# THU-luvision/TextureFusion

Measured on AMD Instinct MI355X. Metric: RGB-D frames/s (TSDF integrate + atlas update: prepare->integrate->finalize, UpdateMeshes, GeneratePatches + UpdateAtlas over the frame's dirty chunks), higher is better.
Workload: dtype f32

## Files before the change

### texturefusion_amd/csrc/tf_kernels.hip

```cpp
#include <stdlib.h>

#include <atomic>
#include "tf_device.h"
#include "tf_devfn.h"
#include "tf_host_math.h"
#include "tf_patch_body.h"
#include "tf_voxel_math.h"

#pragma clang fp contract(off)
#ifndef TF_KA_GP
#define TF_KA_GP 2
#endif


namespace tf {

__global__ void k_reset_ctl(FrameCtl* ctl, VolCtl* vctl) {
  if (blockIdx.x == 0 && threadIdx.x == 0) {
    for (int a = 0; a < 3; ++a) {
      ctl->bbox_key[a] = f2key(1e8f);
      ctl->bbox_key[3 + a] = f2key(-1e8f);
      ctl->min_id[a] = ctl->max_id[a] = ctl->dims[a] = 0;
    }
    ctl->n_coarse = 0;
// ... 497 lines not shown
  auto item_pos = [&](const uint32_t e) -> uint32_t { return FUSED ? list_phys(v, e, nf) : e; };
  const int vy = lane >> 3;
  const int W = cam.W, H = cam.H;
  if (FUSED && bid == 0 && threadIdx.x == 0) {
    for (int a = 0; a < 3; ++a) {
      L.ctl->bbox_key[a] = f2key(1e8f);
      L.ctl->bbox_key[3 + a] = f2key(-1e8f);
    }
  }

  const uint32_t e_first = wave, e_step = nwaves;
  u32x8 rec_next;
  {
    const uint32_t e0 = e_first < n_items ? e_first : 0u;
    const uint32_t p0 = n_items ? item_pos(e0) : 0u;
    rec_next = *(const_u32x8_ptr)(unsigned long long)(&L.list_pre[4 * (p0 < v.max_list ? p0 : 0u)]);
  }

  __shared__ float cenT[3][kChunkVoxels];
  {
    const float4* src = reinterpret_cast<const float4*>(L.cen);
    float4* dst = reinterpret_cast<float4*>(&cenT[0][0]);
    for (int i = threadIdx.x; i < 3 * kChunkVoxels / 4; i += 256) dst[i] = src[i];
  }
  __syncthreads();

  const __amdgpu_buffer_rsrc_t rs_depth =
      __builtin_amdgcn_make_buffer_rsrc((void*)img.depth, 0, W * H * 4, 0x00020000);
  const __amdgpu_buffer_rsrc_t rs_rgba =
      __builtin_amdgcn_make_buffer_rsrc((void*)img.rgba, 0, COLOR ? W * H * 4 : 0, 0x00020000);
  const __amdgpu_buffer_rsrc_t rs_qual =
      __builtin_amdgcn_make_buffer_rsrc((void*)img.quality, 0, QUALITY ? W * H * 4 : 0, 0x00020000);

  const uint32_t row_lo = lane < 32 ? (0xFFu << (lane & 24)) : 0u;
  const uint32_t row_hi = lane < 32 ? 0u : (0xFFu << (lane & 24));
  auto row_any = [&](const unsigned long long m) -> bool {
    return ((((uint32_t)m) & row_lo) | (((uint32_t)(m >> 32)) & row_hi)) != 0u;
  };
  auto ballot = [](const bool b) -> unsigned long long { return __builtin_amdgcn_ballot_w64(b); };

  float c_near = cam.nearP, c_far = cam.farP, c_thr = kc.thrCol, c_lower = kc.lower, c_sigma = kc.sigma;
  asm volatile("" : "+v"(c_near), "+v"(c_far), "+v"(c_thr), "+v"(c_lower), "+v"(c_sigma));

  if (TL && (kc.dbg & 8192u) && lane == 0 && wave < (uint32_t)kPhaseWaves)
  {
    v.phase_buf[wave * 16 + 14] = __builtin_amdgcn_s_memrealtime();
    v.phase_buf[wave * 16 + 8] = 0;
    v.phase_buf[wave * 16 + 9] = 0;
  }

  for (uint32_t e = e_first, e_next = e_first + e_step; e < n_items; e = e_next) {
    const uint32_t pe = item_pos(e);
    const u32x8 prw = rec_next;
    {
      e_next = e + e_step;
      const uint32_t en = e_next < n_items ? e_next : e;
      rec_next = *(const_u32x8_ptr)(unsigned long long)(&L.list_pre[4 * item_pos(en)]);
    }
    const int4 id = make_int4((int)prw[5], (int)prw[6], (int)prw[7], 0);
    const bool owned = part_owned(v, id.x, id.y, id.z);
    if (!owned) {
      if (FUSED && lane == 0) {
        L.list_slot[pe] = kInvalidSlot; L.list_ent[pe] = 0; L.list_new[pe] = 0; L.list_needs[pe] = 0;
        L.list_quality[pe] = 0.0f; L.list_rows[pe] = 0;
      }
      continue;
    }
    const unsigned long long key = pack_id(id.x, id.y, id.z);
    const uint32_t i0 = hash_key(key) & v.hmask;
    u32x4 h0 = {0u, 0u, 0u, 0u};
    uint32_t slot = kInvalidSlot;
    if (FUSED) h0 = *(const_u32x4_ptr)(unsigned long long)(&v.hent[i0]);
    else slot = L.list_slot[pe];
    bool is_new = false;
    uint32_t ent = i0;

    const float o0 = __uint_as_float(prw[0]), o1 = __uint_as_float(prw[1]), o2 = __uint_as_float(prw[2]);
    const float pbx = __uint_as_float(prw[3]), pby = __uint_as_float(prw[4]);
    const f32x2 o01 = {o0, o1};
    const f32x2 fxy = {cam.fxi, cam.fyi}, cxy = {kc.cxs, kc.cys};
    const float wD = FLAG ? pbx : -pbx;
    const float upper = pby;
    const float band = 32.0f * kc.res;
    const bool div_safe = (fabsf(o2) > band) && (fabsf(o2) < 1048576.0f) && (fabsf(o0) < 1048576.0f) &&
                          (fabsf(o1) < 1048576.0f) && (kc.res > 1e-6f) && (kc.res < 16.0f);
    if (TL && (kc.dbg & 8192u) && e == e_first && lane == 0 && wave < (uint32_t)kPhaseWaves) {
      asm volatile("" :: "s"(o0), "s"(o1), "s"(o2), "s"(id.x));
      v.phase_buf[wave * 16 + 15] = __builtin_amdgcn_s_memrealtime();
    }

    int off_d[8];
    int oobl[QUALITY ? 8 : 1];
    int oob_any = 0;
    uint32_t R = 64;
    unsigned long long all_valid = ~0ull;
    uint32_t oob_bits = 0;
    auto geometry = [&](auto safe_tag) {
      constexpr bool SAFE = decltype(safe_tag)::value;
#pragma unroll
      for (int j = 0; j < 8; ++j) {
        const int k = j * 64 + lane;
        const f32x2 pxy = o01 + (f32x2){cenT[0][k], cenT[1][k]};
        const float pzv = o2 + cenT[2][k];
        f32x2 q;
        if (SAFE) {
          q = div2_by(pxy, recip_refined(pzv));
        } else {
          q.x = pxy.x / pzv;
          q.y = pxy.y / pzv;
        }
        const f32x2 uw = q * fxy + cxy;
        const int X = SAFE ? cvt_rne_hw(uw.x) : cvt_sat_rne(uw.x);
        const int Y = SAFE ? cvt_rne_hw(uw.y) : cvt_sat_rne(uw.y);
        const bool valid = ((unsigned)(X - 1) < (unsigned)(W - 2)) && ((unsigned)(Y - 1) < (unsigned)(H - 2));
        all_valid &= ballot(valid);
        int od = (__mul24(Y, W) + X) * 4;
        asm volatile("" : "+v"(od));
        off_d[j] = valid ? od : kOOB;
        if (COLOR) oob_bits |= (((unsigned)X > (unsigned)(W - 1)) || ((unsigned)Y > (unsigned)(H - 1))) ? (1u << j) : 0u;
      }
    };
    if (div_safe) geometry(std::true_type{});
    else geometry(std::false_type{});
    if (QUALITY) {
#pragma unroll
      for (int j = 0; j < 8; ++j) oobl[j] = 0;
    }
    if (all_valid != ~0ull) {
#pragma unroll
      for (int j = 0; j < 8; ++j) {
        if (R == 64u) {
          const unsigned long long vmj = ballot(off_d[j] != kOOB);
          const unsigned long long dead = nonzero_bytes(vmj) ^ 0x0101010101010101ull;
          if (dead) R = (uint32_t)(j * 8) + ((uint32_t)__builtin_ctzll(dead) >> 3);
        }
        const bool live_lane = (uint32_t)(j * 8 + vy) < R;
        if (COLOR) {
          const bool oob = live_lane && ((oob_bits >> j) & 1u);
          oob_any |= oob ? 1 : 0;
          if (QUALITY) oobl[j] = oob ? 1 : 0;
        }
        off_d[j] = live_lane ? off_d[j] : kOOB;
      }
    }

    float dep[8];
#pragma unroll
    for (int j = 0; j < 8; ++j)
      dep[j] = __uint_as_float(__builtin_amdgcn_raw_buffer_load_b32(rs_depth, off_d[j], 0, 0));

    bool lazy_revive = false;
    if (FUSED) {
      if ((((unsigned long long)h0.y << 32) | h0.x) == key && h0.z != kInvalidSlot) {
        slot = h0.z;
        is_new = lazy_revive = (h0.w == 0u);
      } else {
        uint32_t s0 = kInvalidSlot, nw = 1, en = 0;
        if (lane == 0) {
          bool bnew = true;
          s0 = chunk_acquire(v, id, &bnew, &en);
          nw = bnew ? 1u : 0u;
        }
        slot = (uint32_t)__builtin_amdgcn_readfirstlane((int)s0);
        is_new = __builtin_amdgcn_readfirstlane((int)nw) != 0;
        ent = (uint32_t)__builtin_amdgcn_readfirstlane((int)en);
      }
    }
    if (slot == kInvalidSlot) {
      if (FUSED && lane == 0) {
        L.list_slot[pe] = kInvalidSlot; L.list_ent[pe] = 0; L.list_new[pe] = 0; L.list_needs[pe] = 0;
        L.list_quality[pe] = 0.0f; L.list_rows[pe] = 0;
      }
      continue;
    }
    const __amdgpu_buffer_rsrc_t rs_T =
        __builtin_amdgcn_make_buffer_rsrc((void*)(v.tsdf + (size_t)slot * kChunkVoxels), 0, 4096, 0x00020000);
    const __amdgpu_buffer_rsrc_t rs_C =
        __builtin_amdgcn_make_buffer_rsrc((void*)(v.color + (size_t)slot * kChunkVoxels), 0, 4096, 0x00020000);

    float qsum = 0.0f;
    uint32_t lanes_t = 0, lanes_c = 0;
    uint32_t sword = 0;
    unsigned long long m_ok = 0, m_pos = 0, m_neg = 0, m_hvy = 0;

#pragma unroll
    for (int p = 0; p < 8 / GP; ++p) {
      const int g0 = p * GP;
      if ((uint32_t)(g0 * 8) >= R) break;
      float nwv[GP], sd[GP];
      int off_t[GP], off_c[GP], off_i[GP];
      unsigned long long any = 0ull;
#pragma unroll
      for (int j = 0; j < GP; ++j) {
        const int gj = g0 + j;
        const int kb = (gj * 64 + lane) * 8;
        const float d = dep[gj];
        const float s = d - (o2 + cenT[2][gj * 64 + lane]);
        sd[j] = s;
        if (COLOR) {
          const bool upd = (off_d[gj] != kOOB) && (fabsf(s) < c_thr);
          off_i[j] = upd ? off_d[gj] : kOOB;
          const bool ru_l = row_any(ballot(upd));
          const unsigned long long ru = ballot(ru_l);
          off_c[j] = ru_l ? kb : kOOB;
          lanes_c += (uint32_t)__popcll(ru);
          any |= ru;
        }
        const bool act = (uint32_t)(gj * 8 + vy) < R;
        const bool dv = (d > c_near) && (c_far > d);
        const bool inside = (s > c_lower) && (upper > s);
        const bool F = act && dv && inside;
        nwv[j] = F ? wD : 0.0f;
        const bool rf_l = row_any(ballot(F));
        const unsigned long long rf = ballot(rf_l);
        off_t[j] = rf_l ? kb : kOOB;
        lanes_t += (uint32_t)__popcll(rf);
        any |= rf;
      }
      const bool rmw = (any != 0ull) || (COLOR && QUALITY);
      u32x2 t[GP], c[GP];
      uint32_t in[GP];
      float qv[GP];
      if (rmw) {
#pragma unroll
        for (int j = 0; j < GP; ++j) t[j] = __builtin_amdgcn_raw_buffer_load_b64(rs_T, off_t[j], 0, 0);
        if (COLOR) {
#pragma unroll
          for (int j = 0; j < GP; ++j) {
            c[j] = __builtin_amdgcn_raw_buffer_load_b64(rs_C, off_c[j], 0, 0);
            in[j] = __builtin_amdgcn_raw_buffer_load_b32(rs_rgba, off_i[j], 0, 0);
            if (QUALITY) qv[j] = __uint_as_float(__builtin_amdgcn_raw_buffer_load_b32(rs_qual, off_i[j], 0, 0));
          }
        }
      }
      if (rmw) {
#pragma unroll
        for (int j = 0; j < GP; ++j) {
          if (COLOR) {
            const uint32_t p_rg = __builtin_amdgcn_perm(0u, in[j], 0x0c010c00u);
            const uint32_t p_ba = __builtin_amdgcn_perm(0u, in[j], 0x0c030c02u);
            const uint32_t w_rg = c[j].x, w_ba = c[j].y;
            const u16x2 in_rg = __builtin_bit_cast(u16x2, p_rg), in_ba = __builtin_bit_cast(u16x2, p_ba);
            u16x2 c_rg = __builtin_bit_cast(u16x2, w_rg), c_ba = __builtin_bit_cast(u16x2, w_ba);
            if (FLAG) {
              c_rg += in_rg;
              c_ba += in_ba;
              const bool halve = (int)__builtin_bit_cast(uint32_t, c_ba) >= (121 << 16);
              const u16x2 h_rg = c_rg >> (unsigned short)2, h_ba = c_ba >> (unsigned short)2;
              c_rg = halve ? h_rg : c_rg;
              c_ba = halve ? h_ba : c_ba;
            } else {
              c_rg -= in_rg;
              c_ba -= in_ba;
            }
            c[j].x = __builtin_bit_cast(uint32_t, c_rg);
            c[j].y = __builtin_bit_cast(uint32_t, c_ba);
          }
          const float ts = __uint_as_float(t[j].x), tw = __uint_as_float(t[j].y);
          const float nw = nwv[j];
          const float num = ts * tw + sd[j] * nw;
          const float den = (tw + nw) + c_sigma;
          const float ns = num / den;
          const float nwt = tw + nw;
          const bool keep = nwt > 0.5f;
          t[j].x = __float_as_uint(keep ? ns : 999.0f);
          t[j].y = __float_as_uint(keep ? nwt : 0.0f);
        }
      }
      if (rmw) {
#pragma unroll
        for (int j = 0; j < GP; ++j) {
          if (COLOR) __builtin_amdgcn_raw_buffer_store_b64(c[j], rs_C, off_c[j], 0, 0);
          __builtin_amdgcn_raw_buffer_store_b64(t[j], rs_T, off_t[j], 0, 0);
          if (!(kc.dbg & kKaCoarseSumm)) {
            const float fs = __uint_as_float(t[j].x), fw = __uint_as_float(t[j].y);
            const unsigned long long b_ok = ballot(!(fs > 1.0f)), b_pos = ballot(fs > 0.0f) & b_ok;
            const unsigned long long b_neg = ballot(fs < 0.0f), b_hvy = ballot(fw > 50.0f);
            m_ok |= b_ok; m_pos |= b_pos; m_neg |= b_neg; m_hvy |= b_hvy;
            if (g0 + j == 0)
              sword = (b_ok ? 0x1000u : 0u) | (b_pos ? 0x2000u : 0u) | (b_neg ? 0x4000u : 0u) | (b_hvy ? 0x8000u : 0u);
          }
        }
      }
      if (COLOR && QUALITY) {
        const int rowshift = lane & 56;
#pragma unroll
        for (int j = 0; j < GP; ++j) {
          const int gj = g0 + j;
          const unsigned long long mu = ballot(off_i[j] != kOOB);
          const unsigned long long mo = ballot(oobl[gj] != 0);
          if ((mu | mo) == 0ull) continue;
          float rowsum = 0.0f;
          if (mu) {
#pragma unroll
            for (int l = 0; l < 8; ++l) rowsum += __shfl(qv[j], rowshift + l);
          }
          const int left = (int)R - gj * 8;
          const int rmax = left < 8 ? left : 8;
          for (int r = 0; r < rmax; ++r) {
            if ((mo >> (8 * r)) & 0xFFull) qsum = kc.qoob;
            if ((mu >> (8 * r)) & 0xFFull)
              qsum += __int_as_float(__builtin_amdgcn_readlane(__float_as_int(rowsum), 8 * r));
          }
        }
      }
    }
    const uint32_t rows_t = lanes_t >> 3, rows_c = COLOR ? (lanes_c >> 3) : 0u;
    const bool updated = rows_t != 0;
    if (updated) {
      if (kc.dbg & kKaCoarseSumm) {
        if (lane == 0) v.summ[slot] = kSummAny;
      } else {
        const unsigned long long mm[4] = {m_ok, m_pos, m_neg, m_hvy};
#pragma unroll
        for (int b = 0; b < 4; ++b)
          sword |= (mm[b] ? (1u << b) : 0u) | ((mm[b] & 0x0101010101010101ull) ? (0x10u << b) : 0u) | ((mm[b] & 0xFFull) ? (0x100u << b) : 0u);
        if (lane == 0 && sword) atomicOr(&v.summ[slot], sword);
      }
    }
    if (TL && (kc.dbg & 8192u) && lane == 0 && wave < (uint32_t)kPhaseWaves) {
      v.phase_buf[wave * 16 + 8] += 1;
      v.phase_buf[wave * 16 + 9] += rows_t + rows_c;
    }
    if (COLOR && !QUALITY) {
      if (ballot(oob_any != 0) != 0ull) qsum = kc.qoob;
    }

    const bool face = part_band(v, id.x, id.y, id.z);
    if (updated && lane == 0 && (face || lazy_revive)) {
      const uint32_t en = FUSED ? ent : L.list_ent[pe];
      if (face) mark_touched(v, en);
      else v.hent[en].alive = 1u;
    }
    if (FUSED) {
      if (updated) {
        if (lane == 0) v.mark_epoch[slot] = epoch + 1u;
        if (claim_par >= 0) {
          claim_dirty7(v, id, slot, ent, lane, epoch + 1u, claim_par);
        }
      } else if (is_new) {
        if (lane == 0) {
          if (!lazy_revive) v.hent[ent].alive = 0;
          v.mark_epoch[(size_t)v.max_chunks + slot] = epoch + 1u;
        }
        if (rows_c) {
          uint4* c4 = reinterpret_cast<uint4*>(v.color + (size_t)slot * kChunkVoxels);
#pragma unroll
          for (int k = 0; k < 4; ++k) c4[k * 64 + lane] = make_uint4(0, 0, 0, 0);
        }
      }
      if (lane == 0) {
        L.list_slot[pe] = slot;
        L.list_needs[pe] = updated ? 1 : 0;
        L.list_rows[pe] = (uint16_t)(rows_t | (rows_c << 8));
      }
    } else if (lane == 0) {
      if (updated) L.list_needs[pe] = 1;
      L.list_quality[pe] = qsum;
      L.list_rows[pe] = (uint16_t)(rows_t | (rows_c << 8));
    }
  }
}

template <bool COLOR, bool QUALITY, bool FLAG>
__global__ __launch_bounds__(256) void k_integrate(VolumeDev v, FrameImages img, Cam cam, IntegrateConsts kc,
                                                   uint32_t epoch) {
  integrate_body<COLOR, QUALITY, false, FLAG, TF_KA_GP>(v, img, cam, kc, epoch, blockIdx.x, gridDim.x);
}

struct FrameLaunch {
  VolumeDev v;
  FrameImages img;
  Pose P;
  IntegrateConsts kc;
  Cam cam;
  Integ ig;
  uint32_t epoch;
  uint32_t n_ka, n_sel, n_bbox;
  uint32_t rot;
  SelBuf sel1;
  const float* depth1;
  SelectConsts sc1;
  FrameCtl* ctl2;
  const float* depth2;
  Pose P2;
  int claim_par;
  uint32_t n_patch;
  int patch_par;
  KfDev kf_patch;
  uint32_t* progress;
  uint32_t progress_val;
};

template <bool COLOR, bool PATCH, bool TL = false>
__global__ __launch_bounds__(256) __attribute__((amdgpu_waves_per_eu(PATCH ? TF_KFP_WAVES : TF_KF_WAVES, PATCH ? TF_KFP_WAVES : TF_KF_WAVES))) void k_frame(FrameLaunch a) {
  const uint32_t total = a.n_ka + a.n_patch + a.n_sel + a.n_bbox;
  const uint32_t b = blockIdx.x + a.rot < total ? blockIdx.x + a.rot : blockIdx.x + a.rot - total;
  const bool timeline = TL && (a.kc.dbg & 4096u) != 0 && a.n_sel > 0 && a.n_bbox > 0;
  const unsigned long long t0 = timeline ? __builtin_amdgcn_s_memrealtime() : 0ull;
  uint32_t role;
  if (b < a.n_ka) {
    role = 0;
    integrate_body<COLOR, false, true, true, TF_KA_GP, TL>(a.v, a.img, a.cam, a.kc, a.epoch, b, a.n_ka, a.claim_par);
  } else if (PATCH && b < a.n_ka + a.n_patch) {
    role = 3;
    patch_body<true, true, true, TL>(a.v, a.cam, a.patch_par, a.kf_patch, b - a.n_ka, a.n_patch);
  } else if (b < a.n_ka + a.n_patch + a.n_sel) {
    role = 1;
    if (!(TL && (a.kc.dbg & 512u))) {
      VolumeDev v1 = a.v;
      v1.sel = a.sel1;
      select_body<true>(a.depth1, a.cam, a.ig, a.sc1, v1, b - a.n_ka - a.n_patch, a.n_sel);
    }
  } else {
    role = 2;
    if (a.progress && b + 1 == total && threadIdx.x == 0)
      __hip_atomic_store(a.progress, a.progress_val, __ATOMIC_RELAXED, __HIP_MEMORY_SCOPE_SYSTEM);
    if (!(TL && (a.kc.dbg & 1024u))) bbox_body(a.depth2, a.cam, a.P2, a.ctl2, b - a.n_ka - a.n_patch - a.n_sel, a.n_bbox);
  }
// ... 486 lines not shown
```

### texturefusion_amd/csrc/tf_mesh.hip

```cpp
#include <stdlib.h>
#include <string.h>

#include <algorithm>
#include <vector>

#include "tf_devfn.h"
#include "tf_kf_store.h"
#include "tf_mc_table.h"
#include "tf_patch_body.h"
#include "tf_volume.h"

#pragma clang fp contract(off)

namespace tf {

__device__ const unsigned long long d_mc_tri[256] = TF_MC_TRI_TABLE_INIT;

constexpr int kR = 11;
constexpr int kRS = 11;
constexpr int kPS = kRS * kR;
constexpr int kRV = kPS * kR;
constexpr int kEdgeSlots = 3 * 729;
__device__ __forceinline__ uint32_t mesh_shard_rows_d(uint32_t max_chunks) { return max_chunks / kMeshShards + 258u; }

__device__ __forceinline__ int ridx(int x, int y, int z) { return (x + 1) + (y + 1) * kRS + (z + 1) * kPS; }

constexpr bool halo_needed(int rx, int ry, int rz) {
  if (rx < -1 || rx > 9 || ry < -1 || ry > 9 || rz < -1 || rz > 9) return false;
  if (rx >= 0 && rx < 8 && ry >= 0 && ry < 8 && rz >= 0 && rz < 8) return false;
  const int out = ((rx < 0 || rx > 8) ? 1 : 0) + ((ry < 0 || ry > 8) ? 1 : 0) + ((rz < 0 || rz > 8) ? 1 : 0);
  return out <= 1;
}
constexpr int count_halo_pairs() {
  int n = 0;
  for (int rz = -1; rz <= 9; ++rz)
    for (int ry = -1; ry <= 9; ++ry)
      for (int rx = -1; rx <= 9; ++rx) {
        if (!halo_needed(rx, ry, rz)) continue;
        const int vx = (rx + 8) & 7;
        if ((vx & 1) && halo_needed(rx - 1, ry, rz) && (((rx - 1 + 8) >> 3) == ((rx + 8) >> 3))) continue;
        ++n;
      }
  return n;
}
constexpr int kHalo = count_halo_pairs();
struct MeshTabs {
  unsigned long long halo[kHalo];
  uint16_t corner[729];
};
constexpr unsigned long long corner_of(int rx, int ry, int rz) {
  return (rx >= 0 && ry >= 0 && rz >= 0 && rx <= 8 && ry <= 8 && rz <= 8) ? (unsigned long long)(rx + ry * 9 + rz * 81 + 1) : 0ull;
}
constexpr MeshTabs make_mesh_tabs() {
  MeshTabs t{};
  int n = 0;
  for (int rz = -1; rz <= 9; ++rz)
    for (int ry = -1; ry <= 9; ++ry)
      for (int rx = -1; rx <= 9; ++rx) {
        if (!halo_needed(rx, ry, rz)) continue;
        const int vx = (rx + 8) & 7;
        const bool same_chunk_left = ((rx - 1 + 8) >> 3) == ((rx + 8) >> 3);
        if ((vx & 1) && halo_needed(rx - 1, ry, rz) && same_chunk_left) continue;
        const int rx0 = (vx & 1) ? rx - 1 : rx;
        const bool use0 = !(vx & 1);
        const bool use1 = (vx & 1) ? true : (halo_needed(rx + 1, ry, rz) && (((rx + 1 + 8) >> 3) == ((rx + 8) >> 3)));
        const int cx = (rx + 8) >> 3, cy = (ry + 8) >> 3, cz = (rz + 8) >> 3;
        const unsigned long long nb = (unsigned long long)(cx + cy * 3 + cz * 9);
        const unsigned long long pair = (unsigned long long)((((rx0 + 8) & 7) + ((ry + 8) & 7) * 8 + ((rz + 8) & 7) * 64) >> 1);
        const unsigned long long r0 = (unsigned long long)((rx0 + 1) + (ry + 1) * kRS + (rz + 1) * kPS);
        t.halo[n++] = (r0 & 2047ull) | (nb << 11) | (pair << 16) | ((use0 ? 1ull : 0ull) << 24) | ((use1 ? 1ull : 0ull) << 25) |
                      ((use0 ? corner_of(rx0, ry, rz) : 0ull) << 26) | ((use1 ? corner_of(rx0 + 1, ry, rz) : 0ull) << 36);
      }
  for (int c = 0; c < 729; ++c) {
    const int px = c % 9, py = (c / 9) % 9, pz = c / 81;
    t.corner[c] = (uint16_t)((px + 1) + (py + 1) * kRS + (pz + 1) * kPS);
  }
  return t;
}
__device__ const MeshTabs d_mesh_tabs = make_mesh_tabs();

__device__ __forceinline__ int cox(int k) { return (0x66 >> k) & 1; }
__device__ __forceinline__ int coy(int k) { return (0xCC >> k) & 1; }
__device__ __forceinline__ int coz(int k) { return (0xF0 >> k) & 1; }
__device__ __forceinline__ int edge_c0(int e) { return (int)((0x321076543210ull >> (4 * e)) & 0xF); }
__device__ __forceinline__ int edge_c1(int e) { return (int)((0x765447650321ull >> (4 * e)) & 0xF); }

__device__ __forceinline__ int edge_slot(int x, int y, int z, int e) {
  const int bx = x + ((0x622 >> e) & 1);
  const int by = y + ((0xC44 >> e) & 1);
  const int bz = z + ((0x0F0 >> e) & 1);
  const int ax = e >= 8 ? 2 : (e & 1);
  return ax + (bx + by * 9 + bz * 81) * 3;
}
__device__ __forceinline__ int edge_of_slot(int ax, int dx, int dy, int dz) {
  if (ax == 0) return dz ? (dy ? 6 : 4) : (dy ? 2 : 0);
  if (ax == 1) return dz ? (dx ? 5 : 7) : (dx ? 1 : 3);
  return dy ? (dx ? 10 : 11) : (dx ? 9 : 8);
}

__device__ __forceinline__ bool gradient_at(const float* __restrict__ S, int px, int py, int pz, int ox, int oy,
                                            int oz, float res, float g[3]) {
  const int c = ridx(px, py, pz);
  const float xm = S[c - 1], xp = S[c + 1];
  const float ym = S[c - kRS], yp = S[c + kRS];
  const float zm = S[c - kPS], zp = S[c + kPS];
  const bool ok = ((ox ? xp : xm) < 1.0f) && ((oy ? yp : ym) < 1.0f) && ((oz ? zp : zm) < 1.0f);
  const float gx = xp - xm, gy = yp - ym, gz = zp - zm;
  const float yz = gy * gy + gz * gz;
  const float sq = gx * gx + yz;
  const float n = sqrtf(sq);
  g[0] = gx; g[1] = gy; g[2] = gz;
  if (sq > 0.0f) { g[0] = gx / n; g[1] = gy / n; g[2] = gz / n; }
  return ok && !(n > res * 100.0f);
}

constexpr uint32_t kCfHeavy = 64u;
constexpr uint32_t kCfGradOk = 128u;

template <int NT>
struct MeshSh {
  float S[kRV];
  uint8_t cflag[732];
  uint32_t nslot[27];
  unsigned long long rmask[NT];
  uint16_t rbase[NT];
  uint32_t ownq[(kEdgeSlots + 7) / 8];
  uint16_t cinfo[512];
  uint8_t cidx[512];
  uint16_t toff[512];
  uint32_t wsum[8];
  uint32_t nv, nt, adj, any;
  uint32_t ncell;
  uint16_t clist[512];
  uint32_t ovf;
  uint32_t rblock;
  uint32_t rpress;
  uint32_t rstate;
  unsigned long long rtexloc;
};

__device__ __forceinline__ int edge_q(int e) {
  return (int)((0x231023320110ull >> (4 * e)) & 0x3);
}
__device__ __forceinline__ int owner_cell(int m, int q) {
  const int ax = m % 3, b = m / 3;
  const int bx = b % 9, by = (b / 9) % 9, bz = b / 81;
  const int d0 = q & 1, d1 = q >> 1;
  int x, y, z;
  if (ax == 0) { x = bx; y = by - d0; z = bz - d1; }
  else if (ax == 1) { x = bx - d0; y = by; z = bz - d1; }
  else { x = bx - d0; y = by - d1; z = bz; }
  return x + 8 * y + 64 * z;
}

__device__ __forceinline__ void patch_list_append(const VolumeDev& v, int ppar, uint32_t shard, const int4 id,
                                                  uint32_t slot, unsigned long long texloc, uint32_t blk) {
  const uint32_t rows = mesh_shard_rows_d(v.max_chunks);
  const uint32_t p = atomicAdd(&v.patch_cnt[((ppar & 1) * kMeshShards + shard) * 16], 1u);
  const unsigned long long key = pack_id(id.x, id.y, id.z);
  if (p < rows) v.patch_list[((size_t)(ppar & 1) * kMeshShards + shard) * rows + p] = make_int4((int)(uint32_t)key, (int)(uint32_t)(key >> 32), (int)slot, (int)blk);
  else atomicOr(&v.vctl->status, kStMeshFull);
  if (texloc == kNoTexloc) {
    const uint32_t c = atomicAdd(&v.actl->set[ppar & 1].n_cand, 1u);
    if (c < v.max_chunks) v.cand[c] = pack_id(id.x, id.y, id.z);
  }
// ... 320 lines not shown
template <int NT, bool DBG = false>
__global__ __launch_bounds__(NT, TF_MESH_WAVES) void k_mesh(VolumeDev v, const uint32_t* __restrict__ surv, uint32_t* __restrict__ cnt,
                                                 uint32_t* __restrict__ cnt_next, uint32_t cap_sh,
                                                 uint32_t epoch, float res, uint32_t simplified, uint32_t dbg,
                                                 int rearm) {
  __shared__ MeshSh<NT> sh;
  extern __shared__ uint16_t vlist[];
  const int t = threadIdx.x, lane = t & 63;
  uint32_t n_rows = 0, excl_l = 0, incl_l = 0;
  {
    uint32_t my_n = cnt[(lane & 31) * 16 + (lane >> 5)];
    if (my_n > cap_sh) my_n = cap_sh;
    uint32_t incl = my_n;
#pragma unroll
    for (int o = 1; o < 64; o <<= 1) {
      const uint32_t u = (uint32_t)__shfl_up((int)incl, o);
      if (lane >= o) incl += u;
    }
    n_rows = (uint32_t)__builtin_amdgcn_readfirstlane(__shfl((int)incl, 63));
    const uint32_t r0 = blockIdx.x;
    const uint32_t sh0 = (uint32_t)__popcll(__ballot(incl <= r0));
    incl_l = (uint32_t)__builtin_amdgcn_readfirstlane(__shfl((int)incl, (int)(sh0 & 63u)));
    excl_l = incl_l - (uint32_t)__builtin_amdgcn_readfirstlane(__shfl((int)my_n, (int)(sh0 & 63u)));
    incl_l = (uint32_t)__builtin_amdgcn_readfirstlane((int)sh0);
  }
  if (blockIdx.x == 0 && t < (int)kMeshShards) { cnt_next[t * 16] = 0u; cnt_next[t * 16 + 1] = 0u; cnt_next[(kMeshShards + t) * 16] = 0u; cnt_next[(kMeshShards + t) * 16 + 1] = 0u; cnt_next[(2 * kMeshShards + t) * 16] = 0u; }
  if (blockIdx.x < kMeshShards) {
    uint32_t n_reset = cnt[(2u * kMeshShards + blockIdx.x) * 16u];
    if (n_reset > cap_sh) n_reset = cap_sh;
    for (uint32_t i = (uint32_t)t; i < n_reset; i += NT) {
      const int4 e = v.reset_list[(size_t)blockIdx.x * cap_sh + i];
      filter_reset_record(v, (uint32_t)e.w, make_int4(e.x, e.y, e.z, 0), epoch, rearm >= 0 ? (rearm ^ 1) : -1);
    }
  }
  const float half = res * 0.5f;
  if (rearm >= 0 && blockIdx.x == 0 && t == 0) {
    AtlasCtl::Set* O = &v.actl->set[rearm];
    O->n_work = 0; O->n_cand = 0; O->n_patch = 0; O->slots_base = 0ull;
    v.actl->set[rearm ^ 1].slots_base = v.actl->n_slots;
  }
  if (rearm >= 0 && blockIdx.x == 0 && t < (int)kMeshShards) {
    v.patch_cnt[((rearm & 1) * kMeshShards + t) * 16] = 0u;
    v.wl_cnt[((rearm & 1) * kMeshShards + t) * 16] = 0u;
  }
  if (DBG && dbg == 9) mesh_stamp(v, blockIdx.x, 0);
  for (uint32_t r = blockIdx.x; r < n_rows; r += gridDim.x) {
    uint32_t shard, own;
    int4 id;
    float2 a[512 / NT];
    {
      shard = incl_l;
      uint32_t idx = r - excl_l;
      if (r != blockIdx.x) {
        uint32_t my_n = cnt[(lane & 31) * 16 + (lane >> 5)];
        if (my_n > cap_sh) my_n = cap_sh;
        uint32_t incl = my_n;
#pragma unroll
        for (int o = 1; o < 64; o <<= 1) {
          const uint32_t u = (uint32_t)__shfl_up((int)incl, o);
          if (lane >= o) incl += u;
        }
        shard = (uint32_t)__builtin_amdgcn_readfirstlane((int)__popcll(__ballot(incl <= r)));
        idx = r - (uint32_t)__builtin_amdgcn_readfirstlane(__shfl((int)incl, (int)(shard & 63u)) - __shfl((int)my_n, (int)(shard & 63u)));
      }
      if (shard >= kMeshShards) { shard -= kMeshShards; idx = cap_sh - 1u - idx; }
      const size_t row = (size_t)shard * cap_sh + idx;
      own = surv[32 * row + 13];
      id = make_int4((int)surv[32 * row + 27], (int)surv[32 * row + 28], (int)surv[32 * row + 29], 0);
#pragma unroll
      for (int j = 0; j < 512 / NT; ++j) a[j] = v.tsdf[(size_t)own * kChunkVoxels + j * NT + t];
      __syncthreads();
      if (t < 27) sh.nslot[t] = surv[32 * row + t];
    }
    int t_ = threadIdx.x;
    asm volatile("" : "+v"(t_));
    const int t = t_, lane = t & 63, w = t >> 6;
    MeshRec* rec = &v.mesh_rec[own];
    unsigned long long htab[(kHalo + NT - 1) / NT];
#pragma unroll
    for (int j = 0; j < (kHalo + NT - 1) / NT; ++j) htab[j] = (j * NT + t < kHalo) ? d_mesh_tabs.halo[j * NT + t] : ~0ull;
    if (DBG && dbg == 9) mesh_stamp(v, r, 1);
    if (t == 0) { sh.nv = 0; sh.nt = 0; sh.adj = 0; sh.ncell = 0; }
    if (t == NT - 64) { sh.rstate = rec->state; sh.rblock = rec->block; sh.rtexloc = rec->texloc; sh.rpress = blk_pressure(v); }
    if (DBG && dbg == 1) continue;
#pragma unroll
    for (int j = 0; j < 512 / NT; ++j) {
      const int q = j * NT + t;
      const int x0 = q & 7, y0 = (q >> 3) & 7, z0 = q >> 6;
      sh.S[ridx(x0, y0, z0)] = a[j].x; sh.cflag[x0 + y0 * 9 + z0 * 81] = (a[j].y > 50.0f) ? kCfHeavy : 0u;
    }
    __syncthreads();
#pragma unroll
    for (int j = 0; j < (kHalo + NT - 1) / NT; ++j) {
      const unsigned long long e = htab[j];
      if (e == ~0ull) continue;
      const uint32_t s = sh.nslot[(uint32_t)(e >> 11) & 31u];
      float4 val = make_float4(999.0f, 0.0f, 999.0f, 0.0f);
      if (s != kInvalidSlot) val = reinterpret_cast<const float4*>(v.tsdf + (size_t)s * kChunkVoxels)[(uint32_t)(e >> 16) & 255u];
      const uint32_t r0 = (uint32_t)e & 2047u;
      if ((e >> 24) & 1ull) {
        sh.S[r0] = val.x;
        const uint32_t cf = (uint32_t)(e >> 26) & 1023u;
        if (cf) sh.cflag[cf - 1u] = (val.y > 50.0f) ? kCfHeavy : 0u;
      }
      if ((e >> 25) & 1ull) {
        sh.S[r0 + 1u] = val.z;
// ... 155 lines not shown
    const uint32_t nv = sh.nv, nt = sh.nt;
    const uint32_t ovf = sh.ovf;
    if (ovf == kBlkFail) {
      if (t == 0) {
        atomicOr(&v.vctl->status, kStMeshFull);
        const uint32_t was = sh.rstate & kMsInMap;
        rec->nv = 0; rec->nt = 0; rec->state = was | kMsOverflow; rec->epoch = epoch;
        if (rearm >= 0 && was) patch_list_append(v, rearm ^ 1, shard, id, own, sh.rtexloc, sh.rblock);
      }
      __syncthreads();
      continue;
    }
    const uint16_t* const gvlist = (ovf & kBlkLarge) ? v.ovf_vlist + (size_t)((ovf & ~kBlkLarge) - 1u) * kOvfCV : nullptr;

    if (DBG && dbg == 4) continue;
    if (DBG && dbg == 9) mesh_stamp(v, r, 6);
    const uint32_t inmap = (sh.rstate & kMsInMap) | (nv ? kMsInMap : 0u);
    if (t == NT - 64) {
      mesh_block_settle(v, sh.rblock, ovf);
      if (rearm >= 0 && inmap) patch_list_append(v, rearm ^ 1, shard, id, own, sh.rtexloc, ovf);
    }
    const float org[3] = {(float)(8 * id.x) * res, (float)(8 * id.y) * res, (float)(8 * id.z) * res};
    uint32_t adj = 0;
    for (uint32_t i = t; i < nv; i += NT) {
      const int m = gvlist ? gvlist[i] : vlist[i];
      const int cell = owner_cell(m, __builtin_ctz((sh.ownq[m >> 3] >> (4 * (m & 7))) & 0xFu));
      const int x = cell & 7, y = (cell >> 3) & 7, z = cell >> 6;
      const int ax = m % 3, b = m / 3;
      const int bx = b % 9, by = (b / 9) % 9, bz = b / 81;
      const int e = edge_of_slot(ax, bx - x, by - y, bz - z);
      const int e0 = edge_c0(e), e1 = edge_c1(e);
      const float s0 = sh.S[ridx(x + cox(e0), y + coy(e0), z + coz(e0))];
      const float s1 = sh.S[ridx(x + cox(e1), y + coy(e1), z + coz(e1))];
      const float tt = s0 / (s0 - s1);
      const int o0[3] = {cox(e0), coy(e0), coz(e0)}, o1[3] = {cox(e1), coy(e1), coz(e1)};
      const int cc[3] = {x, y, z};
      float pv[3];
#pragma unroll
      for (int a = 0; a < 3; ++a) {
        const float p0 = (float)o0[a] * res, p1 = (float)o1[a] * res;
        const float ev = p0 + tt * (p1 - p0);
        const float origin = org[a] + ((float)cc[a] * res + half);
        pv[a] = ev + origin;
      }
      const int k = (fabsf(s0) > fabsf(s1)) ? e1 : e0;
      const int px = x + cox(k), py = y + coy(k), pz = z + coz(k);
      float g[3];
      gradient_at(sh.S, px, py, pz, cox(k), coy(k), coz(k), res, g);
      const uint32_t cs = sh.nslot[((px + 8) >> 3) + ((py + 8) >> 3) * 3 + ((pz + 8) >> 3) * 9];
      const ushort4 c4 = v.color[(size_t)cs * kChunkVoxels + (px & 7) + (py & 7) * 8 + (pz & 7) * 64];
      float col[3] = {1.0f, 1.0f, 1.0f};
      const float cw = (float)c4.w;
      if (cw > 0.0f) {
        col[0] = ((float)c4.x / 255.0f) / cw;
        col[1] = ((float)c4.y / 255.0f) / cw;
        col[2] = ((float)c4.z / 255.0f) / cw;
      }
#pragma unroll
      for (int a = 0; a < 3; ++a) {
        mesh_plane(v, ovf, kMpPos + a)[i] = pv[a];
        mesh_plane(v, ovf, kMpNrm + a)[i] = g[a];
        mesh_plane(v, ovf, kMpCol + a)[i] = col[a];
        const int gp = (int)floorf((pv[a] - org[a]) / (res * 1.0f));
        if (gp >= 8) adj |= 1u << (2 * a + 1);
        if (gp <= 0) adj |= 1u << (2 * a);
      }
    }
    if (adj) atomicOr(&sh.adj, adj);
    if (DBG && dbg == 9) mesh_stamp(v, r, 7);
    for (uint32_t ci = (uint32_t)(NT - 1 - t); ci < sh.ncell; ci += NT) {
      const int cell = sh.clist[ci];
      const uint32_t info = sh.cinfo[cell];
      if (!(info >> 12)) continue;
      const int x = cell & 7, y = (cell >> 3) & 7, z = cell >> 6;
      const unsigned long long row = d_mc_tri[sh.cidx[cell]];
      const uint32_t valid = info & 0xFFFu;
      uint32_t o = sh.toff[cell];
      for (int col = 0; col < 15; col += 3) {
        const int s0 = (int)((row >> (4 * col)) & 0xF);
        if (s0 == 0xF) break;
        const int s1 = (int)((row >> (4 * col + 4)) & 0xF), s2 = (int)((row >> (4 * col + 8)) & 0xF);
        if (!((valid >> s0) & (valid >> s1) & (valid >> s2) & 1u)) continue;
        constexpr int kEptT = 2304 / NT;
        auto ref_of = [&](int m) {
          const int tt = m / kEptT, j = m - tt * kEptT;
          return (uint16_t)(sh.rbase[tt] + (uint32_t)__popcll(sh.rmask[tt] & ((1ull << j) - 1ull)));
        };
        tri_plane(v, ovf, 0)[o] = ref_of(edge_slot(x, y, z, s2));
        tri_plane(v, ovf, 1)[o] = ref_of(edge_slot(x, y, z, s1));
        tri_plane(v, ovf, 2)[o] = ref_of(edge_slot(x, y, z, s0));
        ++o;
      }
    }
    __syncthreads();
    if (t == 0) {
      rec->nv = (uint16_t)nv; rec->nt = (uint16_t)nt; rec->epoch = epoch; rec->block = ovf;
      rec->state = inmap | (sh.adj << kMsAdjShift) | (inmap ? simplified : 0u);
    }
    __syncthreads();
    if (DBG && dbg == 9) mesh_stamp(v, r, 8);
  }
}

__global__ __launch_bounds__(256) void k_init_mesh_rec(MeshRec* rec, uint32_t n) {
  for (uint32_t i = blockIdx.x * 256 + threadIdx.x; i < n; i += gridDim.x * 256) {
    MeshRec r;
    memset(&r, 0, sizeof(r));
    r.texloc = kNoTexloc;
    r.frameid = -1;
    r.ratio[0] = r.ratio[1] = 1.0f;
    rec[i] = r;
  }
}
void launch_init_meshes(const VolumeDev& v, hipStream_t s) {
  hipLaunchKernelGGL(k_init_mesh_rec, dim3(1024), dim3(256), 0, s, v.mesh_rec, v.max_chunks);
  (void)hipMemsetAsync(v.mesh_rec + v.max_chunks, 0, sizeof(uint32_t) * ((size_t)blk_ring_len(v.mesh_blocks) + blk_ring_len(v.ovf_blocks)), s);
// ... 539 lines not shown
```

### texturefusion_amd/csrc/tf_voxel_math.h

```cpp
#pragma once

#include "tf_devfn.h"
#include "tf_device.h"
#include "tf_host_math.h"

#pragma clang fp contract(off)

namespace tf {

__device__ __forceinline__ int cvt_rne(float x) {
  return (x >= -2147483648.0f && x < 2147483648.0f) ? (int)rintf(x) : (int)0x80000000;
}

__device__ __forceinline__ uint32_t f2key(float f) {
  uint32_t b = __float_as_uint(f);
  return (b & 0x80000000u) ? ~b : (b | 0x80000000u);
}
__device__ __forceinline__ float key2f(uint32_t k) {
  uint32_t b = (k & 0x80000000u) ? (k & 0x7FFFFFFFu) : ~k;
  return __uint_as_float(b);
}

__device__ __forceinline__ float truncation(const Integ& ig, float z) {
  double zz = (double)z * (double)z;
// ... 53 lines not shown
    for (int a = 0; a < 3; ++a) { L.ctl->bbox_key[a] = f2key(1e8f); L.ctl->bbox_key[3 + a] = f2key(-1e8f); }
  }
  for (uint32_t e = bid * 256 + threadIdx.x; e < n; e += nb * 256) {
    const int4 id = L.list_id[e];
    bool is_new = false;
    uint32_t ent = 0;
    const uint32_t slot = chunk_acquire(v, id, &is_new, &ent, lazy);
    L.list_slot[e] = slot;
    L.list_ent[e] = ent;
    L.list_new[e] = is_new ? 1 : 0;
    L.list_needs[e] = 0;
  }
}

__device__ __forceinline__ unsigned long long nonzero_bytes(unsigned long long m) {
  unsigned long long t = m | (m >> 1);
  t |= t >> 2;
  t |= t >> 4;
  return t & 0x0101010101010101ull;
}

typedef unsigned int u32x2 __attribute__((ext_vector_type(2)));
constexpr int kOOB = 0x7FFFFFF0;


__device__ __forceinline__ int cvt_sat_rne(float x) {
  return (int)rintf(__builtin_amdgcn_fmed3f(x, -2147483648.0f, 2147483520.0f));
}

__device__ __forceinline__ int cvt_rne_hw(float x) {
  int r;
  const float n = rintf(x);
  asm("v_cvt_i32_f32_e32 %0, %1" : "=v"(r) : "v"(n));
  return r;
}

struct Recip { float d, r; };
__device__ __forceinline__ Recip recip_refined(float d) {
  Recip R;
  R.d = d;
  const float r0 = __builtin_amdgcn_rcpf(d);
  const float e = __builtin_fmaf(-d, r0, 1.0f);
  R.r = __builtin_fmaf(e, r0, r0);
  return R;
}
typedef float f32x2 __attribute__((ext_vector_type(2)));
__device__ __forceinline__ f32x2 div2_by(const f32x2 n, const Recip& R) {
  const f32x2 d = {-R.d, -R.d}, r = {R.r, R.r};
  const f32x2 q0 = n * r;
  const f32x2 e0 = __builtin_elementwise_fma(d, q0, n);
  const f32x2 q1 = __builtin_elementwise_fma(e0, r, q0);
  const f32x2 e1 = __builtin_elementwise_fma(d, q1, n);
  return __builtin_elementwise_fma(e1, r, q1);
}

typedef unsigned short u16x2 __attribute__((ext_vector_type(2)));

__device__ __forceinline__ void claim_dirty7(const VolumeDev& v, const int4 id, const uint32_t slot, const uint32_t ent, const int lane,
                                             const uint32_t stamp, const int par) {
  uint32_t cs = kInvalidSlot, ce = 0;
  int4 q = id;
  if (lane < 7) {
    q = nbr7(id, lane);
    if (lane == 0) { cs = slot; ce = ent; }
    else if (part_owned(v, q.x, q.y, q.z)) cs = hash_slot_alive_ent(v, pack_id(q.x, q.y, q.z), &ce);
    if (cs != kInvalidSlot && !(atomicMax(&v.mesh_rec[cs].stamp, stamp) < stamp)) cs = kInvalidSlot;
    if (cs != kInvalidSlot) {
      const uint32_t rows = v.max_chunks / kMeshShards + 258u;
      const uint32_t sh = cs & (kMeshShards - 1u);
      const uint32_t p = atomicAdd(&v.wl_cnt[((par & 1) * kMeshShards + sh) * 16], 1u);
      if (p < rows) {
        const size_t at = ((size_t)(par & 1) * kMeshShards + sh) * rows + p;
        v.wl_ids[at] = make_int4(q.x, q.y, q.z, (int)(ce + 1u));
        v.wl_slot[at] = cs;
      } else {
        atomicOr(&v.vctl->status, kStMeshFull);
      }
    }
  }
}

__device__ __forceinline__ unsigned long long obs_pack(uint32_t slot, int32_t kf) {
  return ((unsigned long long)slot << 32) | (unsigned long long)(uint32_t)kf;
}
__device__ __forceinline__ uint32_t obs_find(const VolumeDev& v, unsigned long long key, bool insert) {
  uint32_t i = hash_key(key) & v.obs_mask;
  for (uint32_t probe = 0; probe <= v.obs_mask; ++probe) {
    unsigned long long cur = v.obs_key[i];
    if (cur == kEmptyKey) {
      if (!insert) return kInvalidSlot;
      cur = atomicCAS(&v.obs_key[i], kEmptyKey, key);
      if (cur == kEmptyKey) return i;
    }
    if (cur == key) return i;
    i = (i + 1) & v.obs_mask;
  }
  if (insert) atomicOr(&v.vctl->status, kStHashFull);
  return kInvalidSlot;
}

}
```

Before: 10670.

## Replace IEEE divisions with range-guarded reciprocal-refined fast division paths

Swaps the full-precision division sequences for a reciprocal with FMA Newton refinement in several places: the TSDF update quotient (fused path), mesh normal normalization, color averaging and grid-cell quantization. Each fast path is guarded by a wave-wide ballot that checks operand ranges and falls back to exact division otherwise. The slow fallback paths are rolled into nounroll loops to shrink code size. The next-record prefetch is moved later in the loop body. A waves_per_eu attribute is also added to k_integrate. Rounding could differ slightly from IEEE division, and the range checks add some overhead.

```diff
diff --git a/texturefusion_amd/csrc/tf_kernels.hip b/texturefusion_amd/csrc/tf_kernels.hip
--- a/texturefusion_amd/csrc/tf_kernels.hip
+++ b/texturefusion_amd/csrc/tf_kernels.hip
@@ -573,11 +573,11 @@
   for (uint32_t e = e_first, e_next = e_first + e_step; e < n_items; e = e_next) {
     const uint32_t pe = item_pos(e);
     const u32x8 prw = rec_next;
-    {
-      e_next = e + e_step;
+    e_next = e + e_step;
+    auto request_next = [&]() {
       const uint32_t en = e_next < n_items ? e_next : e;
       rec_next = *(const_u32x8_ptr)(unsigned long long)(&L.list_pre[4 * item_pos(en)]);
-    }
+    };
     const int4 id = make_int4((int)prw[5], (int)prw[6], (int)prw[7], 0);
     const bool owned = part_owned(v, id.x, id.y, id.z);
     if (!owned) {
@@ -585,6 +585,7 @@
         L.list_slot[pe] = kInvalidSlot; L.list_ent[pe] = 0; L.list_new[pe] = 0; L.list_needs[pe] = 0;
         L.list_quality[pe] = 0.0f; L.list_rows[pe] = 0;
       }
+      request_next();
       continue;
     }
     const unsigned long long key = pack_id(id.x, id.y, id.z);
@@ -605,6 +606,7 @@
     const float band = 32.0f * kc.res;
     const bool div_safe = (fabsf(o2) > band) && (fabsf(o2) < 1048576.0f) && (fabsf(o0) < 1048576.0f) &&
                           (fabsf(o1) < 1048576.0f) && (kc.res > 1e-6f) && (kc.res < 16.0f);
+    const bool quot_pre = kc.sigma >= 0.0f;
     if (TL && (kc.dbg & 8192u) && e == e_first && lane == 0 && wave < (uint32_t)kPhaseWaves) {
       asm volatile("" :: "s"(o0), "s"(o1), "s"(o2), "s"(id.x));
       v.phase_buf[wave * 16 + 15] = __builtin_amdgcn_s_memrealtime();
@@ -627,8 +629,13 @@
         if (SAFE) {
           q = div2_by(pxy, recip_refined(pzv));
         } else {
-          q.x = pxy.x / pzv;
-          q.y = pxy.y / pzv;
+          q = (f32x2){0.0f, 0.0f};
+#pragma nounroll
+          for (int it = 0; it < 2; ++it) {
+            const float r = (it ? pxy.y : pxy.x) / pzv;
+            q.x = it ? q.x : r;
+            q.y = it ? r : q.y;
+          }
         }
         const f32x2 uw = q * fxy + cxy;
         const int X = SAFE ? cvt_rne_hw(uw.x) : cvt_sat_rne(uw.x);
@@ -692,6 +699,7 @@
         L.list_slot[pe] = kInvalidSlot; L.list_ent[pe] = 0; L.list_new[pe] = 0; L.list_needs[pe] = 0;
         L.list_quality[pe] = 0.0f; L.list_rows[pe] = 0;
       }
+      request_next();
       continue;
     }
     const __amdgpu_buffer_rsrc_t rs_T =
@@ -777,15 +785,36 @@
             c[j].x = __builtin_bit_cast(uint32_t, c_rg);
             c[j].y = __builtin_bit_cast(uint32_t, c_ba);
           }
-          const float ts = __uint_as_float(t[j].x), tw = __uint_as_float(t[j].y);
-          const float nw = nwv[j];
-          const float num = ts * tw + sd[j] * nw;
-          const float den = (tw + nw) + c_sigma;
-          const float ns = num / den;
-          const float nwt = tw + nw;
-          const bool keep = nwt > 0.5f;
-          t[j].x = __float_as_uint(keep ? ns : 999.0f);
-          t[j].y = __float_as_uint(keep ? nwt : 0.0f);
+        }
+        if (FUSED) {
+          float num[GP], den[GP], ns[GP];
+          bool keep[GP];
+#pragma unroll
+          for (int j = 0; j < GP; ++j) {
+            const float ts = __uint_as_float(t[j].x), tw = __uint_as_float(t[j].y);
+            const float nw = nwv[j];
+            num[j] = ts * tw + sd[j] * nw;
+            den[j] = (tw + nw) + c_sigma;
+            const float nwt = tw + nw;
+            keep[j] = nwt > 0.5f;
+            t[j].y = __float_as_uint(keep[j] ? nwt : 0.0f);
+          }
+          quot_kept<GP>(ns, num, den, keep, quot_pre);
+#pragma unroll
+          for (int j = 0; j < GP; ++j) t[j].x = __float_as_uint(keep[j] ? ns[j] : 999.0f);
+        } else {
+#pragma unroll
+          for (int j = 0; j < GP; ++j) {
+            const float ts = __uint_as_float(t[j].x), tw = __uint_as_float(t[j].y);
+            const float nw = nwv[j];
+            const float num = ts * tw + sd[j] * nw;
+            const float den = (tw + nw) + c_sigma;
+            const float ns = num / den;
+            const float nwt = tw + nw;
+            const bool keep = nwt > 0.5f;
+            t[j].x = __float_as_uint(keep ? ns : 999.0f);
+            t[j].y = __float_as_uint(keep ? nwt : 0.0f);
+          }
         }
       }
       if (rmw) {
@@ -826,20 +855,24 @@
         }
       }
     }
+    request_next();
+    const int lane_t = (int)__builtin_amdgcn_mbcnt_hi(~0u, __builtin_amdgcn_mbcnt_lo(~0u, 0u));
+    uint32_t ep1 = epoch + 1u;
+    asm volatile("" : "+s"(ep1));
     const uint32_t rows_t = lanes_t >> 3, rows_c = COLOR ? (lanes_c >> 3) : 0u;
     const bool updated = rows_t != 0;
     if (updated) {
       if (kc.dbg & kKaCoarseSumm) {
-        if (lane == 0) v.summ[slot] = kSummAny;
+        if (lane_t == 0) v.summ[slot] = kSummAny;
       } else {
         const unsigned long long mm[4] = {m_ok, m_pos, m_neg, m_hvy};
 #pragma unroll
         for (int b = 0; b < 4; ++b)
           sword |= (mm[b] ? (1u << b) : 0u) | ((mm[b] & 0x0101010101010101ull) ? (0x10u << b) : 0u) | ((mm[b] & 0xFFull) ? (0x100u << b) : 0u);
-        if (lane == 0 && sword) atomicOr(&v.summ[slot], sword);
-      }
-    }
-    if (TL && (kc.dbg & 8192u) && lane == 0 && wave < (uint32_t)kPhaseWaves) {
+        if (lane_t == 0 && sword) atomicOr(&v.summ[slot], sword);
+      }
+    }
+    if (TL && (kc.dbg & 8192u) && lane_t == 0 && wave < (uint32_t)kPhaseWaves) {
       v.phase_buf[wave * 16 + 8] += 1;
       v.phase_buf[wave * 16 + 9] += rows_t + rows_c;
     }
@@ -848,34 +881,34 @@
     }
 
     const bool face = part_band(v, id.x, id.y, id.z);
-    if (updated && lane == 0 && (face || lazy_revive)) {
+    if (updated && lane_t == 0 && (face || lazy_revive)) {
       const uint32_t en = FUSED ? ent : L.list_ent[pe];
       if (face) mark_touched(v, en);
       else v.hent[en].alive = 1u;
     }
     if (FUSED) {
       if (updated) {
-        if (lane == 0) v.mark_epoch[slot] = epoch + 1u;
+        if (lane_t == 0) v.mark_epoch[slot] = ep1;
         if (claim_par >= 0) {
-          claim_dirty7(v, id, slot, ent, lane, epoch + 1u, claim_par);
+          claim_dirty7(v, id, slot, ent, lane_t, ep1, claim_par);
         }
       } else if (is_new) {
-        if (lane == 0) {
+        if (lane_t == 0) {
           if (!lazy_revive) v.hent[ent].alive = 0;
-          v.mark_epoch[(size_t)v.max_chunks + slot] = epoch + 1u;
+          v.mark_epoch[(size_t)v.max_chunks + slot] = ep1;
         }
         if (rows_c) {
           uint4* c4 = reinterpret_cast<uint4*>(v.color + (size_t)slot * kChunkVoxels);
 #pragma unroll
-          for (int k = 0; k < 4; ++k) c4[k * 64 + lane] = make_uint4(0, 0, 0, 0);
-        }
-      }
-      if (lane == 0) {
+          for (int k = 0; k < 4; ++k) c4[k * 64 + lane_t] = make_uint4(0, 0, 0, 0);
+        }
+      }
+      if (lane_t == 0) {
         L.list_slot[pe] = slot;
         L.list_needs[pe] = updated ? 1 : 0;
         L.list_rows[pe] = (uint16_t)(rows_t | (rows_c << 8));
       }
-    } else if (lane == 0) {
+    } else if (lane_t == 0) {
       if (updated) L.list_needs[pe] = 1;
       L.list_quality[pe] = qsum;
       L.list_rows[pe] = (uint16_t)(rows_t | (rows_c << 8));
@@ -884,8 +917,8 @@
 }
 
 template <bool COLOR, bool QUALITY, bool FLAG>
-__global__ __launch_bounds__(256) void k_integrate(VolumeDev v, FrameImages img, Cam cam, IntegrateConsts kc,
-                                                   uint32_t epoch) {
+__global__ __launch_bounds__(256) __attribute__((amdgpu_waves_per_eu(TF_KF_WAVES, TF_KF_WAVES))) void k_integrate(VolumeDev v, FrameImages img, Cam cam,
+                                                                                                                IntegrateConsts kc, uint32_t epoch) {
   integrate_body<COLOR, QUALITY, false, FLAG, TF_KA_GP>(v, img, cam, kc, epoch, blockIdx.x, gridDim.x);
 }
 
diff --git a/texturefusion_amd/csrc/tf_mesh.hip b/texturefusion_amd/csrc/tf_mesh.hip
--- a/texturefusion_amd/csrc/tf_mesh.hip
+++ b/texturefusion_amd/csrc/tf_mesh.hip
@@ -9,6 +9,7 @@
 #include "tf_mc_table.h"
 #include "tf_patch_body.h"
 #include "tf_volume.h"
+#include "tf_voxel_math.h"
 
 #pragma clang fp contract(off)
 
@@ -110,7 +111,16 @@
   const float sq = gx * gx + yz;
   const float n = sqrtf(sq);
   g[0] = gx; g[1] = gy; g[2] = gz;
-  if (sq > 0.0f) { g[0] = gx / n; g[1] = gy / n; g[2] = gz / n; }
+  if (sq > 0.0f) {
+    auto comp_ok = [](const float c) { return __float_as_uint(c) == 0u || fabsf(c) >= 5.42101086242752217e-20f; };
+    const bool in = (n >= 2.3283064365386963e-10f) && (n < 4294967296.0f) && comp_ok(gx) && comp_ok(gy) && comp_ok(gz);
+    if (__builtin_amdgcn_ballot_w64(!in) == 0ull) {
+      const Recip R = recip_refined(n);
+      g[0] = div_by(gx, R); g[1] = div_by(gy, R); g[2] = div_by(gz, R);
+    } else {
+      g[0] = gx / n; g[1] = gy / n; g[2] = gz / n;
+    }
+  }
   return ok && !(n > res * 100.0f);
 }
 
@@ -537,6 +547,8 @@
       shard = incl_l;
       uint32_t idx = r - excl_l;
       if (r != blockIdx.x) {
+        int lane = threadIdx.x & 63;
+        asm volatile("" : "+v"(lane));
         uint32_t my_n = cnt[(lane & 31) * 16 + (lane >> 5)];
         if (my_n > cap_sh) my_n = cap_sh;
         uint32_t incl = my_n;
@@ -798,16 +810,29 @@
       float col[3] = {1.0f, 1.0f, 1.0f};
       const float cw = (float)c4.w;
       if (cw > 0.0f) {
-        col[0] = ((float)c4.x / 255.0f) / cw;
-        col[1] = ((float)c4.y / 255.0f) / cw;
-        col[2] = ((float)c4.z / 255.0f) / cw;
+        const Recip R255 = {255.0f, 0x1.010102p-8f}, Rcw = recip_refined(cw);
+        col[0] = div_by(div_by((float)c4.x, R255), Rcw);
+        col[1] = div_by(div_by((float)c4.y, R255), Rcw);
+        col[2] = div_by(div_by((float)c4.z, R255), Rcw);
+      }
+      float rel[3], gq[3];
+#pragma unroll
+      for (int a = 0; a < 3; ++a) rel[a] = pv[a] - org[a];
+      const bool rel_in = (fabsf(rel[0]) < 1099511627776.0f) && (fabsf(rel[1]) < 1099511627776.0f) && (fabsf(rel[2]) < 1099511627776.0f);
+      if (res > 1e-6f && res < 16.0f && __builtin_amdgcn_ballot_w64(!rel_in) == 0ull) {
+        const Recip Rres = recip_refined(res * 1.0f);
+#pragma unroll
+        for (int a = 0; a < 3; ++a) gq[a] = div_by(rel[a], Rres);
+      } else {
+#pragma unroll
+        for (int a = 0; a < 3; ++a) gq[a] = rel[a] / (res * 1.0f);
       }
 #pragma unroll
       for (int a = 0; a < 3; ++a) {
         mesh_plane(v, ovf, kMpPos + a)[i] = pv[a];
         mesh_plane(v, ovf, kMpNrm + a)[i] = g[a];
         mesh_plane(v, ovf, kMpCol + a)[i] = col[a];
-        const int gp = (int)floorf((pv[a] - org[a]) / (res * 1.0f));
+        const int gp = (int)floorf(gq[a]);
         if (gp >= 8) adj |= 1u << (2 * a + 1);
         if (gp <= 0) adj |= 1u << (2 * a);
       }
diff --git a/texturefusion_amd/csrc/tf_voxel_math.h b/texturefusion_amd/csrc/tf_voxel_math.h
--- a/texturefusion_amd/csrc/tf_voxel_math.h
+++ b/texturefusion_amd/csrc/tf_voxel_math.h
@@ -129,6 +129,60 @@
   const f32x2 q1 = __builtin_elementwise_fma(e0, r, q0);
   const f32x2 e1 = __builtin_elementwise_fma(d, q1, n);
   return __builtin_elementwise_fma(e1, r, q1);
+}
+
+__device__ __forceinline__ float div_by(const float n, const Recip& R) {
+  const float q0 = n * R.r;
+  const float e0 = __builtin_fmaf(-R.d, q0, n);
+  const float q1 = __builtin_fmaf(e0, R.r, q0);
+  const float e1 = __builtin_fmaf(-R.d, q1, n);
+  return __builtin_fmaf(e1, R.r, q1);
+}
+
+constexpr float kQuotDenHi = 4294967296.0f;
+constexpr float kQuotNumLo = 5.42101086242752217e-20f;
+constexpr float kQuotNumHi = 18446744073709551616.0f;
+__device__ __forceinline__ bool quot_in_range(const float num, const float den) {
+  const float an = fabsf(num);
+  return (den < kQuotDenHi) && (an >= kQuotNumLo) && (an < kQuotNumHi);
+}
+template <int N>
+__device__ __forceinline__ void quot_kept(float (&q)[N], const float (&num)[N], const float (&den)[N], const bool (&kept)[N],
+                                          const bool pre, bool* fast = nullptr) {
+  bool out = false;
+#pragma unroll
+  for (int j = 0; j < N; ++j) out |= kept[j] && !quot_in_range(num[j], den[j]);
+  const bool go = pre && __builtin_amdgcn_ballot_w64(out) == 0ull;
+  if (fast) *fast = go;
+  if (go) {
+#pragma unroll
+    for (int j = 0; j + 1 < N; j += 2) {
+      const f32x2 d = {-den[j], -den[j + 1]}, n = {num[j], num[j + 1]};
+      const f32x2 r0 = {__builtin_amdgcn_rcpf(den[j]), __builtin_amdgcn_rcpf(den[j + 1])};
+      const f32x2 e = __builtin_elementwise_fma(d, r0, (f32x2){1.0f, 1.0f});
+      const f32x2 r = __builtin_elementwise_fma(e, r0, r0);
+      const f32x2 q0 = n * r;
+      const f32x2 e0 = __builtin_elementwise_fma(d, q0, n);
+      const f32x2 q1 = __builtin_elementwise_fma(e0, r, q0);
+      const f32x2 e1 = __builtin_elementwise_fma(d, q1, n);
+      const f32x2 qq = __builtin_elementwise_fma(e1, r, q1);
+      q[j] = qq.x;
+      q[j + 1] = qq.y;
+    }
+    if (N & 1) q[N - 1] = div_by(num[N - 1], recip_refined(den[N - 1]));
+  } else {
+#pragma unroll
+    for (int j = 0; j < N; ++j) q[j] = 0.0f;
+#pragma nounroll
+    for (int it = 0; it < N; ++it) {
+      float a = num[0], b = den[0];
+#pragma unroll
+      for (int j = 1; j < N; ++j) { a = it == j ? num[j] : a; b = it == j ? den[j] : b; }
+      const float r = a / b;
+#pragma unroll
+      for (int j = 0; j < N; ++j) q[j] = it == j ? r : q[j];
+    }
+  }
 }
 
 typedef unsigned short u16x2 __attribute__((ext_vector_type(2)));
```

After: 10440. 2.2% lower.
